# BerkIGuler/AdaFortiTran

Hardware: AMD Instinct MI355X
Metric: OFDM frames/sec (120x14 grid, batch 128) + channel-estimation MSE vs reference (higher is better)
Workload: dtype f32; 1 GPU; C3: AdaFortiTran default config (6 layers, d=128, 4 heads, adaptive tokens), 120x14 grid, pilots 12x2; 128 frames per GPU per step; step = model(pilots_cpu, meta_cpu) through the module surface + device MSE partial; value = SURVEY 8(d)'s metric: H2D of pilots + meta INSIDE the step, output left on the device (= value_h2d_inclusive); the bare engine call on inputs resident in HBM is value_resident;; frames_per_gpu=128, global_batch=128, parallelism=frames sharded over 1 rank(s), lanes=1

## Files before the change

adafortitran_amd/csrc/k_misc.hip:

```cpp
#include <algorithm>

#include "aft_internal.h"
#include "conv_device.h"
#include "pack_device.h"

namespace aft {

struct AdapterArgs {
    const float *cond[3];
    const float *w[3][3], *b[3][3];
    float *tokens6;
    int h0, h1, h2, tokens;
};

__device__ __forceinline__ void adapter_body(const AdapterArgs &a, int b, int e, float *sm) {
    float *a0 = sm, *a1 = sm + a.h0;
    const int tid = threadIdx.x;
    const float x = a.cond[e][b];
    constexpr int kH0Max = 8, kPer2 = 3;
    const bool fast = a.h0 <= kH0Max && a.h1 == 42 && a.h2 <= kPer2 * 256 && a.h1 <= 256;
    if (fast) {
        float w0 = 0.f, b0 = 0.f, w1[kH0Max], b1 = 0.f, b2[kPer2];
        f32x2 w2[kPer2][21];
        if (tid < a.h0) { w0 = a.w[e][0][tid]; b0 = a.b[e][0][tid]; }
#pragma unroll
        for (int k = 0; k < kH0Max; ++k) w1[k] = (tid < a.h1 && k < a.h0) ? a.w[e][1][tid * a.h0 + k] : 0.f;
        if (tid < a.h1) b1 = a.b[e][1][tid];
#pragma unroll
        for (int u = 0; u < kPer2; ++u) {
            const int i = tid + 256 * u;
            const bool ok = i < a.h2;
            const float *wr = a.w[e][2] + (size_t)(ok ? i : 0) * 42;
#pragma unroll
            for (int k = 0; k < 21; ++k) w2[u][k] = *reinterpret_cast<const f32x2 *>(wr + 2 * k);
            b2[u] = ok ? a.b[e][2][i] : 0.f;
        }
        if (tid < a.h0) a0[tid] = fmaxf(fmaf(w0, x, b0), 0.f);
        __syncthreads();
        if (tid < a.h1) {
            float acc = b1;
#pragma unroll
            for (int k = 0; k < kH0Max; ++k)
                if (k < a.h0) acc = fmaf(w1[k], a0[k], acc);
            a1[tid] = fmaxf(acc, 0.f);
        }
        __syncthreads();
#pragma unroll
        for (int u = 0; u < kPer2; ++u) {
            const int i = tid + 256 * u;
            if (i >= a.h2) break;
            float acc = b2[u];
#pragma unroll
            for (int k = 0; k < 21; ++k) {
                acc = fmaf(w2[u][k][0], a1[2 * k], acc);
                acc = fmaf(w2[u][k][1], a1[2 * k + 1], acc);
            }
            a.tokens6[((size_t)b * a.tokens + (i >> 1)) * 6 + 2 * e + (i & 1)] = acc;
        }
        return;
    }
    for (int i = tid; i < a.h0; i += 256) a0[i] = fmaxf(fmaf(a.w[e][0][i], x, a.b[e][0][i]), 0.f);
    __syncthreads();
    for (int i = tid; i < a.h1; i += 256) {
        float acc = a.b[e][1][i];
        for (int k = 0; k < a.h0; ++k) acc = fmaf(a.w[e][1][i * a.h0 + k], a0[k], acc);
        a1[i] = fmaxf(acc, 0.f);
    }
    __syncthreads();
    for (int i = tid; i < a.h2; i += 256) {
        float acc = a.b[e][2][i];
        const float *wr = a.w[e][2] + (size_t)i * a.h1;
        for (int k = 0; k < a.h1; ++k) acc = fmaf(wr[k], a1[k], acc);
        a.tokens6[((size_t)b * a.tokens + (i >> 1)) * 6 + 2 * e + (i & 1)] = acc;
    }
}

__global__ __launch_bounds__(256) void adapter_kernel(const AdapterArgs a) {
    extern __shared__ float sm[];
    adapter_body(a, blockIdx.x, blockIdx.y, sm);
}

static AdapterArgs adapter_args(const aft_config &c, const WeightsDev &w, const float *snr, const float *ds,
                                const float *dop, float *tokens6) {
    AdapterArgs a{};
    a.cond[0] = snr; a.cond[1] = ds; a.cond[2] = dop;
    for (int e = 0; e < 3; ++e)
        for (int j = 0; j < 3; ++j) { a.w[e][j] = w.ada_w[e][j]; a.b[e][j] = w.ada_b[e][j]; }
    a.tokens6 = tokens6;
    a.h0 = c.hidden[0]; a.h1 = c.hidden[1]; a.h2 = c.hidden[2];
    a.tokens = (c.num_scs / c.patch_scs) * (c.num_symbols / c.patch_symbols);
    return a;
}

hipError_t launch_adapter(const aft_config &c, const WeightsDev &w, const float *snr, const float *ds,
                          const float *dop, float *tokens6, int batch, hipStream_t st) {
    const AdapterArgs a = adapter_args(c, w, snr, ds, dop, tokens6);
    hipLaunchKernelGGL(adapter_kernel, dim3(batch, 3), dim3(256), sizeof(float) * (a.h0 + a.h1), st, a);
    return hipGetLastError();
}


constexpr int kFoldTok = 2, kFoldChunk = 16;
struct FoldArgs {
    const float *wkv, *bv;
    const float *w1, *b1, *pos;
    float *tk, *tvt, *wf;
    int d, K, tokens, tokpad;
};
inline size_t fold_tables_lds(int d) { return sizeof(float) * ((size_t)256 * (kFoldChunk + 1) + (size_t)kFoldTok * d); }

__device__ __forceinline__ void fold_tables_body(const FoldArgs &f, int blk, float *sm) {
    float *sw = sm, *sc = sm + 256 * (kFoldChunk + 1);
    const int tid = threadIdx.x, chunks = (2 * f.d + 255) / 256;
    const int t0 = (blk / chunks) * kFoldTok, row0 = (blk % chunks) * 256, row = row0 + tid;
    for (int i = tid; i < kFoldTok * f.d; i += 256) {
        const int tt = i / f.d, k = i - tt * f.d, t = t0 + tt;
        sc[i] = t < f.tokens ? f.b1[k] + f.pos[(size_t)t * f.d + k] : 0.f;
    }
    float acc[kFoldTok];
#pragma unroll
    for (int tt = 0; tt < kFoldTok; ++tt) acc[tt] = row >= f.d && row < 2 * f.d ? f.bv[row - f.d] : 0.f;
    constexpr int kPieces = kFoldChunk / 4;
    f32x4 piece[kPieces];
    auto request = [&](int kc) {
#pragma unroll
        for (int m = 0; m < kPieces; ++m) {
            const int i = tid + 256 * m, rr = i / kPieces, c4 = (i % kPieces) * 4;
            piece[m] = f32x4{0.f, 0.f, 0.f, 0.f};
            if (row0 + rr < 2 * f.d) piece[m] = *reinterpret_cast<const f32x4 *>(f.wkv + (size_t)(row0 + rr) * f.d + kc + c4);
        }
    };
    request(0);
    for (int kc = 0; kc < f.d; kc += kFoldChunk) {
        __syncthreads();
#pragma unroll
        for (int m = 0; m < kPieces; ++m) {
            const int i = tid + 256 * m, rr = i / kPieces, c4 = (i % kPieces) * 4;
#pragma unroll
            for (int j = 0; j < 4; ++j) sw[rr * (kFoldChunk + 1) + c4 + j] = piece[m][j];
        }
        if (kc + kFoldChunk < f.d) request(kc + kFoldChunk);
        __syncthreads();
#pragma unroll
        for (int kk = 0; kk < kFoldChunk; ++kk) {
            const float wv = sw[tid * (kFoldChunk + 1) + kk];
#pragma unroll
            for (int tt = 0; tt < kFoldTok; ++tt) acc[tt] = fmaf(wv, sc[tt * f.d + kc + kk], acc[tt]);
        }
    }
#pragma unroll
    for (int tt = 0; tt < kFoldTok; ++tt) {
        const int t = t0 + tt;
        if (row < f.d) {
            if (t < f.tokens) f.tk[(size_t)t * f.d + row] = acc[tt];
        } else if (row < 2 * f.d && t < f.tokpad) {
            f.tvt[(size_t)(row - f.d) * f.tokpad + t] = t < f.tokens ? acc[tt] : 0.f;
        }
    }
}

__device__ __forceinline__ void fold_matrices_body(const FoldArgs &f, int blk) {
    const int o = blk * 256 + threadIdx.x, per_part = (f.d / 32) * kFoldSteps * 64;
    if (o >= 2 * per_part) return;
    const int part = o / per_part, rem = o - part * per_part;
    const int wblock = rem / (kFoldSteps * 64), st = rem / 64 % kFoldSteps, lane = rem & 63;
    const int row = part * f.d + 32 * wblock + (lane & 31), k = 2 * st + (lane >> 5);
    float acc = 0.f;
    if (k < f.K) {
        const float *wr = f.wkv + (size_t)row * f.d;
        for (int j = 0; j < f.d; j += 4) {
            const f32x4 wv = *reinterpret_cast<const f32x4 *>(wr + j);
#pragma unroll
            for (int jj = 0; jj < 4; ++jj) acc = fmaf(wv[jj], f.w1[(size_t)(j + jj) * f.K + k], acc);
        }
    }
    f.wf[o] = acc;
}

struct PrologueArgs {
    AdapterArgs ad;
    float *packed;
    const float *pilots;
    float *up_planes;
    int adapter_blocks, pack_blocks, d, num_layers, split;
    int up_bx, npix, pf, nplanes;
    float *conv_frag;
    int frag_blocks;
    FoldArgs fold;
    int fold_table_blocks, fold_matrix_blocks;
};

__global__ __launch_bounds__(256) void prologue_kernel(const WeightsDev w, const PrologueArgs a) {
    extern __shared__ __attribute__((aligned(16))) float sm[];
    int blk = blockIdx.x;
    if (blk < a.adapter_blocks) {
        adapter_body(a.ad, blk / 3, blk % 3, sm);
        return;
    }
    blk -= a.adapter_blocks;
    if (blk < a.fold_table_blocks) {
        fold_tables_body(a.fold, blk, sm);
        return;
    }
    blk -= a.fold_table_blocks;
    if (blk < a.fold_matrix_blocks) {
        fold_matrices_body(a.fold, blk);
        return;
    }
    blk -= a.fold_matrix_blocks;
    if (blk < a.pack_blocks) {
        const size_t v = (size_t)blk * 256 + threadIdx.x, dd4 = (size_t)a.d * a.d / 4;
        if (a.fold_table_blocks > 0 && v >= dd4 && v < 3 * dd4) return;
        pack_weights_vec(w, a.packed, a.d, 0, a.num_layers, a.split, v);
        return;
    }
    blk -= a.pack_blocks;
    if (blk < a.frag_blocks) {
        const int v = blk * 256 + threadIdx.x;
        constexpr int kPerStack = kFragFloats / 4;
        if (v < 2 * kPerStack) {
            const int stack = v / kPerStack, rem = v - stack * kPerStack;
            const float *const *cw = stack ? w.ref_w : w.enh_w;
            const float *const *cb = stack ? w.ref_b : w.enh_b;
            f32x4 o;
            if (rem < kFragQuads * 64) {
                const int quad = rem >> 6, lane = rem & 63;
#pragma unroll
                for (int jj = 0; jj < 4; ++jj) o[jj] = conv_frag16_entry(cw[1], cb[1], cw[2], cb[2], 4 * quad + jj, lane);
            } else {
                const int i0 = 4 * (rem - kFragQuads * 64), h = i0 / 80;
#pragma unroll
                for (int jj = 0; jj < 4; ++jj) o[jj] = conv_helper_entry(cw[0], cb[0], cw[3], cb[3], h, i0 - 80 * h + jj);
            }
            *reinterpret_cast<f32x4 *>(a.conv_frag + (size_t)v * 4) = o;
        }
        return;
    }
    blk -= a.frag_blocks;
    upsample_planes_body(sm, w.up_w, w.up_b, a.pilots, a.up_planes, a.npix, a.pf, a.nplanes, blk % a.up_bx, blk / a.up_bx);
}

bool prologue_upsample_ok(const aft_config &c, const WeightsDev &w) {
    return upsample_planes_ok(w.up_w, c.pilot_scs * c.pilot_symbols);
}

hipError_t launch_prologue(const aft_config &c, const WeightsDev &w, const float *snr, const float *ds, const float *dop,
                           float *tokens6, int batch, float *packed, const float *pilots, float *up_planes, hipStream_t st,
                           float *conv_frag, const L0Fold *fold) {
    PrologueArgs a{};
    if (conv_frag != nullptr) {
        a.conv_frag = conv_frag;
        a.frag_blocks = (2 * (kFragFloats / 4) + 255) / 256;
    }
    size_t lds = 0;
    if (c.adaptive) {
        a.ad = adapter_args(c, w, snr, ds, dop, tokens6);
        a.adapter_blocks = 3 * batch;
        lds = sizeof(float) * (a.ad.h0 + a.ad.h1);
    }
    if (packed != nullptr) {
        a.packed = packed; a.d = c.model_dim; a.num_layers = std::min(c.num_layers, kLayerWindow);
        a.split = c.precision == AFT_PRECISION_BF16X3 ? 1 : 0;
        a.pack_blocks = (int)((packed_layer_floats(c.model_dim) * a.num_layers / 4 + 255) / 256);
    }
    int up_blocks = 0;
    if (up_planes != nullptr && prologue_upsample_ok(c, w)) {
        a.pilots = pilots; a.up_planes = up_planes;
        a.npix = c.num_scs * c.num_symbols; a.pf = c.pilot_scs * c.pilot_symbols; a.nplanes = 2 * batch;
        a.up_bx = (a.npix + kUpPix - 1) / kUpPix;
        up_blocks = a.up_bx * ((a.nplanes + kUpPlanes - 1) / kUpPlanes);
        lds = std::max(lds, upsample_planes_lds(a.pf));
    }
    if (fold != nullptr && fold->tk != nullptr) {
        FoldArgs &f = a.fold;
        f.d = c.model_dim; f.K = c.patch_scs * c.patch_symbols + (c.adaptive ? 6 : 0);
        f.tokens = tokens_of(c); f.tokpad = round_up(f.tokens, kTile);
        f.wkv = w.layers[0].in_proj_w + (size_t)f.d * f.d; f.bv = w.layers[0].in_proj_b + 2 * f.d;
        f.w1 = w.lin1_w; f.b1 = w.lin1_b; f.pos = w.pos;
        f.tk = fold->tk; f.tvt = fold->tvt; f.wf = fold->wf;
        a.d = c.model_dim;
        a.fold_table_blocks = (f.tokpad + kFoldTok - 1) / kFoldTok * ((2 * f.d + 255) / 256);
        a.fold_matrix_blocks = (2 * (f.d / 32) * kFoldSteps * 64 + 255) / 256;
        lds = std::max(lds, fold_tables_lds(f.d));
    }
    const int blocks = a.adapter_blocks + a.fold_table_blocks + a.fold_matrix_blocks + a.pack_blocks + a.frag_blocks + up_blocks;
    if (blocks == 0) return hipSuccess;
    hipLaunchKernelGGL(prologue_kernel, dim3(blocks), dim3(256), lds, st, w, a);
    return hipGetLastError();
}

struct EmbedArgs {
    const float *conv_enhanced, *tokens6, *w1, *b1, *pos;
    float *x;
    int S, T, p0, p1, tokens, d, din, planes;
};

template <int D, bool ADAPTIVE, int PMAX>
__global__ __launch_bounds__(256) void embed_kernel(const EmbedArgs a) {
    constexpr int PER = D / 32, NF = ADAPTIVE ? PMAX + 6 : PMAX;
    const int tid = threadIdx.x, hw = tid >> 5, lane32 = tid & 31;
    const int tw = a.T / a.p1, p = a.p0 * a.p1;
    extern __shared__ float sm[];
    for (int i = tid; i < a.din * D; i += 256) sm[(i % a.din) * D + i / a.din] = a.w1[i];
    __syncthreads();
    float w[NF][PER], b1[PER];
#pragma unroll
    for (int f = 0; f < NF; ++f) {
        const int frow = f < PMAX ? f : p + (f - PMAX);
#pragma unroll
        for (int i = 0; i < PER; ++i) w[f][i] = (f < PMAX && f >= p) ? 0.f : sm[frow * D + lane32 * PER + i];
    }
#pragma unroll
    for (int i = 0; i < PER; ++i) b1[i] = a.b1[lane32 * PER + i];
    const unsigned rows = (unsigned)a.planes * a.tokens, rstep = gridDim.x * 8u, tokens = a.tokens;
    const unsigned dn = rstep / tokens, dt = rstep % tokens;
    int poff[PMAX];
#pragma unroll
    for (int f = 0; f < PMAX; ++f) poff[f] = (f / a.p1) * a.T + f % a.p1;
    struct Tok { unsigned row, n, t; };
    auto advance = [&](Tok k) {
        k.row += rstep; k.n += dn; k.t += dt;
        if (k.t >= tokens) { k.t -= tokens; ++k.n; }
        return k;
    };
    auto fetch = [&](const Tok &k, float (&vin)[NF], float (&ps)[PER]) {
        const unsigned tq = k.t / (unsigned)tw, tr = k.t - tq * tw;
        const float *ce = a.conv_enhanced + ((size_t)k.n * a.S + tq * a.p0) * a.T + tr * a.p1;
#pragma unroll
        for (int f = 0; f < PMAX; ++f) vin[f] = f < p ? ce[poff[f]] : 0.f;
        if constexpr (ADAPTIVE) {
            const float *tk = a.tokens6 + ((size_t)(k.n >> 1) * tokens + k.t) * 6;
#pragma unroll
            for (int f = 0; f < 6; ++f) vin[PMAX + f] = tk[f];
        }
#pragma unroll
        for (int i = 0; i < PER; ++i) ps[i] = a.pos[k.t * D + lane32 * PER + i];
    };
    auto emit = [&](const Tok &k, const float (&vin)[NF], const float (&ps)[PER]) {
        float acc[PER];
#pragma unroll
        for (int i = 0; i < PER; ++i) acc[i] = b1[i] + ps[i];
#pragma unroll
        for (int f = 0; f < NF; ++f)
#pragma unroll
            for (int i = 0; i < PER; ++i) acc[i] = fmaf(w[f][i], vin[f], acc[i]);
#pragma unroll
        for (int i = 0; i < PER; ++i) a.x[(size_t)k.row * D + lane32 * PER + i] = acc[i];
    };
    float va[NF], pa[PER], vb[NF], pb[PER];
    Tok k0;
    k0.row = blockIdx.x * 8u + hw;
    k0.n = k0.row / tokens;
    k0.t = k0.row - k0.n * tokens;
    if (k0.row < rows) fetch(k0, va, pa);
    while (k0.row < rows) {
        const Tok k1 = advance(k0), k2 = advance(k1);
        if (k1.row < rows) fetch(k1, vb, pb);
        emit(k0, va, pa);
        if (k1.row < rows) {
            if (k2.row < rows) fetch(k2, va, pa);
            emit(k1, vb, pb);
        }
        k0 = k2;
    }
}

hipError_t launch_embed(const aft_config &c, const WeightsDev &w, const float *conv_enhanced, const float *tokens6,
                        float *x, int batch, hipStream_t st) {
    EmbedArgs a{};
    a.conv_enhanced = conv_enhanced; a.tokens6 = tokens6;
    a.w1 = w.lin1_w; a.b1 = w.lin1_b; a.pos = w.pos; a.x = x;
    a.S = c.num_scs; a.T = c.num_symbols; a.p0 = c.patch_scs; a.p1 = c.patch_symbols;
    a.tokens = (a.S / a.p0) * (a.T / a.p1);
    a.d = c.model_dim;
    a.din = a.p0 * a.p1 + (c.adaptive ? 6 : 0);
    a.planes = 2 * batch;
    const long rows = (long)a.planes * a.tokens;
    const int blocks = (int)std::min<long>((rows + 7) / 8, 1024);
    const size_t lds = sizeof(float) * a.din * a.d;
    const bool small = a.p0 * a.p1 <= 6;
    if (a.p0 * a.p1 > kMaxPatchFeatures) return hipErrorInvalidValue;
#define AFT_EMBED(D_, A_)                                                                              \
    do {                                                                                               \
        if (small) hipLaunchKernelGGL((embed_kernel<D_, A_, 6>), dim3(blocks), dim3(256), lds, st, a); \
        else hipLaunchKernelGGL((embed_kernel<D_, A_, kMaxPatchFeatures>), dim3(blocks), dim3(256), lds, st, a); \
    } while (0)
    if (c.model_dim == 32 && c.adaptive) AFT_EMBED(32, true);
    else if (c.model_dim == 32) AFT_EMBED(32, false);
    else if (c.model_dim == 96 && c.adaptive) AFT_EMBED(96, true);
    else if (c.model_dim == 96) AFT_EMBED(96, false);
    else if (c.model_dim == 160 && c.adaptive) AFT_EMBED(160, true);
    else if (c.model_dim == 160) AFT_EMBED(160, false);
    else if (c.model_dim == 224 && c.adaptive) AFT_EMBED(224, true);
    else if (c.model_dim == 224) AFT_EMBED(224, false);
    else if (c.model_dim == 64 && c.adaptive) AFT_EMBED(64, true);
    else if (c.model_dim == 64) AFT_EMBED(64, false);
    else if (c.model_dim == 128 && c.adaptive) AFT_EMBED(128, true);
    else if (c.model_dim == 128) AFT_EMBED(128, false);
    else if (c.model_dim == 192 && c.adaptive) AFT_EMBED(192, true);
    else if (c.model_dim == 192) AFT_EMBED(192, false);
    else if (c.model_dim == 256 && c.adaptive) AFT_EMBED(256, true);
    else if (c.model_dim == 256) AFT_EMBED(256, false);
    else return hipErrorInvalidValue;
#undef AFT_EMBED
    return hipGetLastError();
}

__global__ __launch_bounds__(256) void linear_kernel(const float *__restrict__ w, const float *__restrict__ bias,
                                                     const float *__restrict__ pilots, float *__restrict__ out,
                                                     int in_f, int out_f) {
    extern __shared__ float sm[];
    const int b = blockIdx.y;
    for (int i = threadIdx.x; i < 2 * in_f; i += 256) sm[i] = pilots[(size_t)b * 2 * in_f + i];
    __syncthreads();
    const int o = blockIdx.x * 256 + threadIdx.x;
    if (o >= out_f) return;
    const float bv = bias != nullptr ? bias[o] : 0.f;
    float re = bv, im = bv;
    const float *wr = w + (size_t)o * in_f;
    for (int k = 0; k < in_f; ++k) {
        re = fmaf(wr[k], sm[2 * k], re);
        im = fmaf(wr[k], sm[2 * k + 1], im);
    }
    *reinterpret_cast<float2 *>(out + ((size_t)b * out_f + o) * 2) = make_float2(re, im);
}

hipError_t launch_linear(const float *weight, const float *bias, const float *pilots, float *out, int batch,
                         int in_features, int out_features, hipStream_t st) {
    hipLaunchKernelGGL(linear_kernel, dim3((out_features + 255) / 256, batch), dim3(256),
                       sizeof(float) * 2 * in_features, st, weight, bias, pilots, out, in_features, out_features);
    return hipGetLastError();
}

__global__ __launch_bounds__(256) void mse_kernel(const float *__restrict__ est, const float *__restrict__ ref,
                                                  double *sum_sq, long long n_floats) {
    double acc = 0.0;
    const long long n4 = n_floats / 4;
    const long long stride = (long long)gridDim.x * 256;
    for (long long i = (long long)blockIdx.x * 256 + threadIdx.x; i < n4; i += stride) {
        const f32x4 e = reinterpret_cast<const f32x4 *>(est)[i];
        const f32x4 r = reinterpret_cast<const f32x4 *>(ref)[i];
#pragma unroll
        for (int j = 0; j < 4; ++j) {
            const float dlt = e[j] - r[j];
            acc += (double)dlt * (double)dlt;
        }
    }
    if (blockIdx.x == 0)
        for (long long i = n4 * 4 + threadIdx.x; i < n_floats; i += 256) {
            const float dlt = est[i] - ref[i];
            acc += (double)dlt * (double)dlt;
        }
#pragma unroll
    for (int o = 32; o >= 1; o >>= 1) acc += __shfl_xor(acc, o);
    __shared__ double part[4];
    if ((threadIdx.x & 63) == 0) part[threadIdx.x >> 6] = acc;
    __syncthreads();
    if (threadIdx.x == 0) atomicAdd(sum_sq, part[0] + part[1] + part[2] + part[3]);
}

hipError_t launch_mse(const float *est, const float *ref, double *sum_sq, long long n_complex, hipStream_t st) {
    const long long n_floats = 2 * n_complex;
    long long blocks = (n_floats / 4 + 255) / 256;
    if (blocks < 1) blocks = 1;
    if (blocks > 128) blocks = 128;
    hipLaunchKernelGGL(mse_kernel, dim3((int)blocks), dim3(256), 0, st, est, ref, sum_sq, n_floats);
    return hipGetLastError();
}

__global__ __launch_bounds__(256) void pilot_gather_kernel(const float2 *__restrict__ grid, float2 *__restrict__ pilots,
                                                           int *__restrict__ counts, int batch, int n, int expected) {
    const int lane = threadIdx.x & 63;
    const int frame = blockIdx.x * 4 + (threadIdx.x >> 6);
    if (frame >= batch) return;
    const float2 *src = grid + (size_t)frame * n;
    int base = 0;
    for (int i0 = 0; i0 < n; i0 += 8 * 64) {
        float2 v[8];
#pragma unroll
        for (int u = 0; u < 8; ++u) {
            const int i = i0 + 64 * u + lane;
            v[u] = i < n ? src[i] : make_float2(0.f, 0.f);
        }
#pragma unroll
        for (int u = 0; u < 8; ++u) {
            const bool nz = v[u].x != 0.f || v[u].y != 0.f;
            const unsigned long long m = __ballot(nz);
            const int pos = base + __popcll(m & ((1ull << lane) - 1ull));
            if (nz && pos < expected) pilots[(size_t)frame * expected + pos] = v[u];
            base += __popcll(m);
        }
    }
    for (int pos = base + lane; pos < expected; pos += 64)
        pilots[(size_t)frame * expected + pos] = make_float2(0.f, 0.f);
    if (lane == 0) counts[frame] = base;
}

hipError_t launch_pilot_gather(const float *hzero_ls, float *pilots, int *counts, int batch, int grid_elems,
                               int expected, hipStream_t st) {
    hipLaunchKernelGGL(pilot_gather_kernel, dim3((batch + 3) / 4), dim3(256), 0, st,
                       reinterpret_cast<const float2 *>(hzero_ls), reinterpret_cast<float2 *>(pilots), counts, batch,
                       grid_elems, expected);
    return hipGetLastError();
}

constexpr int kGatherLoads = 4, kGatherPiece = 64 * kGatherLoads;

struct FrameGatherArgs {
    const float *src[2];
    float *dst[2];
    const long long *index;
    int *flags;
    long long frames;
    unsigned waves, per_frame;
    int elems[2];
    int nvec[2], pieces[2];
    int wide[2];
};

template <typename V>
__device__ __forceinline__ void gather_piece(const float *src, float *dst, int nvec, int piece, int lane, bool ok) {
    V *d = reinterpret_cast<V *>(dst);
    const int i0 = piece * kGatherPiece + lane;
    if (ok) {
        const V *s = reinterpret_cast<const V *>(src);
        V v[kGatherLoads];
#pragma unroll
        for (int u = 0; u < kGatherLoads; ++u) v[u] = s[min(i0 + 64 * u, nvec - 1)];
#pragma unroll
        for (int u = 0; u < kGatherLoads; ++u) {
            const int i = i0 + 64 * u;
            if (i < nvec) d[i] = v[u];
        }
    } else {
#pragma unroll
        for (int u = 0; u < kGatherLoads; ++u) {
            const int i = i0 + 64 * u;
            if (i < nvec) d[i] = V{};
        }
    }
}

__global__ __launch_bounds__(256) void frame_gather_kernel(const FrameGatherArgs a) {
    const int lane = threadIdx.x & 63;
    const unsigned wave = __builtin_amdgcn_readfirstlane((int)(threadIdx.x >> 6)) + blockIdx.x * (blockDim.x >> 6);
    if (wave >= a.waves) return;
    const unsigned b = wave / a.per_frame;
    int piece = (int)(wave - b * a.per_frame);
    const int arr = piece < a.pieces[0] ? 0 : 1;
    if (arr) piece -= a.pieces[0];
    const long long idx = a.index[b];
    const bool ok = (unsigned long long)idx < (unsigned long long)a.frames;
    if (arr == 0 && piece == 0 && lane == 0) a.flags[b] = ok ? 0 : 1;
    const size_t fl = 2 * (size_t)a.elems[arr];
    const float *src = a.src[arr] + (ok ? (size_t)idx * fl : 0);
    float *dst = a.dst[arr] + (size_t)b * fl;
    if (a.wide[arr]) gather_piece<f32x4>(src, dst, a.nvec[arr], piece, lane, ok);
    else gather_piece<f32x2>(src, dst, a.nvec[arr], piece, lane, ok);
}

hipError_t launch_frame_gather(const float *ideal_all, const float *pilots_all, const long long *index, float *ideal_out,
                               float *pilots_out, int *flags, int batch, long long frames, int grid_elems, int pilot_elems,
                               hipStream_t st) {
    FrameGatherArgs a{};
    a.src[0] = ideal_all; a.src[1] = pilots_all; a.dst[0] = ideal_out; a.dst[1] = pilots_out;
    a.index = index; a.flags = flags; a.frames = frames;
    a.elems[0] = grid_elems; a.elems[1] = pilot_elems;
    for (int k = 0; k < 2; ++k) {
        const bool wide = a.elems[k] % 2 == 0 && (reinterpret_cast<uintptr_t>(a.src[k]) | reinterpret_cast<uintptr_t>(a.dst[k])) % 16 == 0;
        a.wide[k] = wide ? 1 : 0;
        a.nvec[k] = wide ? a.elems[k] / 2 : a.elems[k];
        a.pieces[k] = (a.nvec[k] + kGatherPiece - 1) / kGatherPiece;
    }
    a.per_frame = (unsigned)(a.pieces[0] + a.pieces[1]);
    const long long waves = (long long)batch * a.per_frame;
    if (waves > 0x7fffffffLL) return hipErrorInvalidValue;
    a.waves = (unsigned)waves;
    const int wpb = waves < 4LL * current_device_cus() ? 1 : 4;
    const long long blocks = (waves + wpb - 1) / wpb;
    hipLaunchKernelGGL(frame_gather_kernel, dim3((unsigned)blocks), dim3(64 * wpb), 0, st, a);
    return hipGetLastError();
}

constexpr int kEmbAnyRows = 8, kEmbAnyDin = kMaxPatchGeneral + 6;
__global__ __launch_bounds__(256) void embed_any_kernel(const EmbedArgs a) {
    __shared__ float in[kEmbAnyRows][kEmbAnyDin];
    const int tid = threadIdx.x, tw = a.T / a.p1, p = a.p0 * a.p1;
    const long rows = (long)a.planes * a.tokens, row0 = (long)blockIdx.x * kEmbAnyRows;
    for (int i = tid; i < kEmbAnyRows * kEmbAnyDin; i += 256) {
        const int r = i / kEmbAnyDin, f = i - r * kEmbAnyDin;
        const long row = row0 + r;
        float v = 0.f;
#ifdef AFT_TEST_LDS_BUG
        if (f >= a.din) continue;
#endif
        if (row < rows && f < a.din) {
            const int n = (int)(row / a.tokens), t = (int)(row - (long)n * a.tokens);
            if (f < p) {
                const int tq = t / tw, tr = t - tq * tw;
                v = a.conv_enhanced[((size_t)n * a.S + tq * a.p0 + f / a.p1) * a.T + tr * a.p1 + f % a.p1];
            } else {
                v = a.tokens6[((size_t)(n >> 1) * a.tokens + t) * 6 + (f - p)];
            }
        }
        in[r][f] = v;
    }
    __syncthreads();
    for (int c = tid; c < a.d; c += 256) {
        float w[kEmbAnyDin];
#pragma unroll
        for (int f = 0; f < kEmbAnyDin; ++f) w[f] = f < a.din ? a.w1[(size_t)c * a.din + f] : 0.f;
        const float b = a.b1[c];
        for (int r = 0; r < kEmbAnyRows; ++r) {
            const long row = row0 + r;
            if (row >= rows) break;
            const int t = (int)(row % a.tokens);
            float acc = b + a.pos[(size_t)t * a.d + c];
#pragma unroll
            for (int f = 0; f < kEmbAnyDin; ++f) acc = fmaf(w[f], in[r][f], acc);
            a.x[(size_t)row * a.d + c] = acc;
        }
    }
}

hipError_t launch_embed_any(const aft_config &c, const WeightsDev &w, const float *conv_enhanced, const float *tokens6,
                            float *x, int batch, hipStream_t st) {
    EmbedArgs a{};
    a.conv_enhanced = conv_enhanced; a.tokens6 = tokens6;
    a.w1 = w.lin1_w; a.b1 = w.lin1_b; a.pos = w.pos; a.x = x;
    a.S = c.num_scs; a.T = c.num_symbols; a.p0 = c.patch_scs; a.p1 = c.patch_symbols;
    a.tokens = (a.S / a.p0) * (a.T / a.p1);
    a.d = c.model_dim;
    a.din = a.p0 * a.p1 + (c.adaptive ? 6 : 0);
    a.planes = 2 * batch;
    if (a.p0 * a.p1 > kMaxPatchGeneral || (c.adaptive && tokens6 == nullptr)) return hipErrorInvalidValue;
    if (!switch_on(SW_EMBED_ANY_OLD) && ends_train_ok(a.planes, a.S, a.T, a.p0, a.p1, a.d, c.adaptive != 0))
        return launch_embed_train_fwd(conv_enhanced, c.adaptive ? tokens6 : nullptr, w.lin1_w, w.lin1_b, w.pos, x, a.planes, a.S, a.T, a.p0,
                                      a.p1, a.d, st, true);
    const long rows = (long)a.planes * a.tokens;
    hipLaunchKernelGGL(embed_any_kernel, dim3((unsigned)((rows + kEmbAnyRows - 1) / kEmbAnyRows)), dim3(256), 0, st, a);
    return hipGetLastError();
}

__global__ __launch_bounds__(1024) void fill_lds_kernel(float value, float *sink) {
    extern __shared__ __attribute__((aligned(16))) float lds_all[];
    constexpr int kFloats = 160 * 1024 / 4;
    for (int i = threadIdx.x; i < kFloats; i += 1024) lds_all[i] = value;
    __syncthreads();
    const unsigned long long t0 = __builtin_amdgcn_s_memtime();
    while (__builtin_amdgcn_s_memtime() - t0 < 20000) __builtin_amdgcn_s_sleep(16);
    if (sink != nullptr && lds_all[(threadIdx.x * 977) % kFloats] == 12345.678f) *sink = 1.f;
}
__global__ __launch_bounds__(256) void peek_lds_kernel(float *__restrict__ out, int n) {
    extern __shared__ __attribute__((aligned(16))) float lds_peek[];
    for (int i = threadIdx.x; i < n; i += 256) out[(size_t)blockIdx.x * n + i] = lds_peek[i];
}
hipError_t launch_peek_lds(float *out, int workgroups, int n, hipStream_t st) {
    hipLaunchKernelGGL(peek_lds_kernel, dim3(workgroups), dim3(256), 40 * 1024, st, out, n);
    return hipGetLastError();
}
hipError_t launch_fill_lds(float value, hipStream_t st) {
    static PerDeviceOnce attr;
    hipError_t e = ensure_dynamic_lds(attr, reinterpret_cast<const void *>(fill_lds_kernel), 160 * 1024);
    if (e != hipSuccess) return e;
    hipLaunchKernelGGL(fill_lds_kernel, dim3(4 * current_device_cus()), dim3(1024), 160 * 1024, st, value, (float *)nullptr);
    return hipGetLastError();
}

__global__ __launch_bounds__(256) void ls_mse_db_kernel(const float2 *__restrict__ ls, const float2 *__restrict__ ideal,
                                                        float *__restrict__ db, int batch, int n) {
    const int lane = threadIdx.x & 63;
    const int frame = blockIdx.x * 4 + (threadIdx.x >> 6);
    if (frame >= batch) return;
    double acc = 0.0;
    for (int i = lane; i < n; i += 64) {
        const float2 a = ls[(size_t)frame * n + i], b = ideal[(size_t)frame * n + i];
        const double dr = (double)a.x - (double)b.x, di = (double)a.y - (double)b.y;
        acc += dr * dr + di * di;
    }
#pragma unroll
    for (int o = 32; o >= 1; o >>= 1) acc += __shfl_xor(acc, o);
    if (lane == 0) db[frame] = (float)(10.0 * log10(acc / (double)n));
}

hipError_t launch_ls_mse_db(const float *ls, const float *ideal, float *db, int batch, int grid_elems, hipStream_t st) {
    hipLaunchKernelGGL(ls_mse_db_kernel, dim3((batch + 3) / 4), dim3(256), 0, st, reinterpret_cast<const float2 *>(ls),
                       reinterpret_cast<const float2 *>(ideal), db, batch, grid_elems);
    return hipGetLastError();
}

}
```

adafortitran_amd/csrc/switches.h:

```cpp
#pragma once

#define AFT_SWITCHES(X) \
    X(LANES, "AFT_LANES", "1 = never split a forward into lanes; 2 .. 4 = always that many shares (header section \"Lanes\")") \
    X(L0_FOLD, "AFT_L0_FOLD", "0 = layer 0's keys and values by the model_dim-deep product over x0, not from the input features on the prologue's tables (DESIGN.md 4.1)") \
    X(LAYER_FUSED, "AFT_LAYER_FUSED", "0 = never the one-launch-per-layer sequence (k_layer.hip), 1 = wherever its shape is covered (default: where plane-aligned tiles add no round)") \
    X(PROLOGUE_NO_UP, "AFT_PROLOGUE_NO_UP", "measurement: the profiled prologue launch without the pilot upsampler product") \
    X(CONV_NSPLIT, "AFT_CONV_NSPLIT", "1 | 2 | 4 column ranges per plane in the streaming conv kernels (default: by the batch)") \
    X(CONV_BANDED, "AFT_CONV_BANDED", "the banded conv kernel instead of the column- / row-streaming ones") \
    X(CONV_COLUMN_TILES, "AFT_CONV_COLUMN_TILES", "the column-tiled conv path even where a band plan fits; n > 2 = at least n tiles per plane") \
    X(GEMM_BM, "AFT_GEMM_BM", "64 | 96: row tile of the training GEMM (default: by the shape)") \
    X(EMBED_ANY_OLD, "AFT_EMBED_ANY_OLD", "the general engine's own embedding kernel instead of the training path's") \
    X(EMBED_BWD_GENERIC, "AFT_EMBED_BWD_GENERIC", "the vector embedding backward instead of the MFMA one (model_dim 128)") \
    X(TRAIN_UNFUSED_FWD, "AFT_TRAIN_UNFUSED_FWD", "the launch sequence the fused forward chain of a training layer replaced") \
    X(TRAIN_UNFUSED_BWD, "AFT_TRAIN_UNFUSED_BWD", "the launch sequence the fused backward chain of a training layer replaced") \
    X(TRAIN_ATTN_BWD_SPLIT, "AFT_TRAIN_ATTN_BWD_SPLIT", "the two-pass attention backward instead of the one-pass kernel") \
    X(ATTN_BWD_GROUPS, "AFT_ATTN_BWD_GROUPS", "1 | 4 problems per workgroup of the one-pass attention backward (default: by shape)") \
    X(STAMPS, "AFT_STAMPS", "phase stamps printed on the host: the diag variant only (libaft_hip_diag.so, build.build_diag(): -DAFT_DIAG_STAMPS)") \
    X(ALLOW_COMPOSITE, "AFT_ALLOW_COMPOSITE", "1 = run a configuration the kernels do not cover on the PyTorch-ROCm composite") \
    X(TRAIN_NO_FUSED_ENDS, "AFT_TRAIN_NO_FUSED_ENDS", "training: PyTorch's unfold / cat / add around the dense ends, not fused") \
    X(TRAIN_NO_QKV_CHAIN, "AFT_TRAIN_NO_QKV_CHAIN", "training: every layer runs its own in-projection GEMM (no chained tapes)") \
    X(PRECISION, "AFT_PRECISION", "f32 | bf16x3: the estimators' default hip_precision") \
    X(ENCODER_PATH, "AFT_ENCODER_PATH", "auto | launches | plane: aft_config.encoder_path of every HipEngine (`plane`: retired, runs the launches)")

namespace aft {

enum Switch : int {
#define AFT_SWITCH_ID(id, name, purpose) SW_##id,
    AFT_SWITCHES(AFT_SWITCH_ID)
#undef AFT_SWITCH_ID
    kNumSwitches
};

bool switch_on(Switch s);
int switch_int(Switch s, int dflt);

}
```

Before: 85520 frames/s.

## Compute layer-0 fold tables and matrices with MFMA tiles in the prologue

```diff
diff --git a/adafortitran_amd/csrc/k_misc.hip b/adafortitran_amd/csrc/k_misc.hip
--- a/adafortitran_amd/csrc/k_misc.hip
+++ b/adafortitran_amd/csrc/k_misc.hip
@@ -177,6 +177,109 @@
     f.wf[o] = acc;
 }
 
+__device__ __forceinline__ f32x4 fold_steps_of(f32x4 x) {
+    using u32x2 = __attribute__((ext_vector_type(2))) unsigned;
+    unsigned r[4];
+#pragma unroll
+    for (int c = 0; c < 4; ++c) { const float v = x[c]; r[c] = __builtin_bit_cast(unsigned, v); }
+    u32x2 p = __builtin_amdgcn_permlane32_swap(r[0], r[2], false, false);
+    r[0] = p[0]; r[2] = p[1];
+    p = __builtin_amdgcn_permlane32_swap(r[1], r[3], false, false);
+    r[1] = p[0]; r[3] = p[1];
+    p = __builtin_amdgcn_permlane16_swap(r[0], r[1], false, false);
+    r[0] = p[0]; r[1] = p[1];
+    p = __builtin_amdgcn_permlane16_swap(r[2], r[3], false, false);
+    r[2] = p[0]; r[3] = p[1];
+    return f32x4{__builtin_bit_cast(float, r[0]), __builtin_bit_cast(float, r[1]), __builtin_bit_cast(float, r[2]), __builtin_bit_cast(float, r[3])};
+}
+
+template <int NS, bool TABLE>
+__device__ __forceinline__ f32x4 fold_chain(const float *ap, const float *bp, int bstep, const float *cp, f32x4 acc, int blocks) {
+    constexpr int NQ = NS / 4;
+    for (int kb = 0; kb < blocks; ++kb) {
+        f32x4 av[NQ], bw[NQ], cw[NQ];
+        float bs[NS];
+#pragma unroll
+        for (int j = 0; j < NQ; ++j) av[j] = *reinterpret_cast<const f32x4 *>(ap + 16 * j);
+        if constexpr (TABLE) {
+#pragma unroll
+            for (int j = 0; j < NQ; ++j) bw[j] = *reinterpret_cast<const f32x4 *>(bp + 16 * j);
+#pragma unroll
+            for (int j = 0; j < NQ; ++j) cw[j] = *reinterpret_cast<const f32x4 *>(cp + 16 * j);
+        } else {
+#pragma unroll
+            for (int s = 0; s < NS; ++s) bs[s] = bp[(size_t)s * bstep];
+        }
+        __builtin_amdgcn_sched_barrier(0);
+#pragma unroll
+        for (int j = 0; j < NQ; ++j) {
+            const f32x4 a4 = fold_steps_of(av[j]);
+            f32x4 b4;
+            if constexpr (TABLE) b4 = fold_steps_of(cw[j] + bw[j]);
+            else b4 = f32x4{bs[4 * j], bs[4 * j + 1], bs[4 * j + 2], bs[4 * j + 3]};
+#pragma unroll
+            for (int m = 0; m < 4; ++m) acc = __builtin_amdgcn_mfma_f32_16x16x4f32(a4[m], b4[m], acc, 0, 0, 0);
+        }
+        ap += 4 * NS; bp += TABLE ? (size_t)4 * NS : (size_t)NS * bstep; cp += 4 * NS;
+    }
+    return acc;
+}
+template <bool TABLE>
+__device__ __forceinline__ f32x4 fold_chain_d(int d, const float *ap, const float *bp, int bstep, const float *cp, f32x4 acc) {
+    switch (d >> 5) {
+        case 1: return fold_chain<8, TABLE>(ap, bp, bstep, cp, acc, 1);
+        case 2: return fold_chain<16, TABLE>(ap, bp, bstep, cp, acc, 1);
+        case 3: return fold_chain<24, TABLE>(ap, bp, bstep, cp, acc, 1);
+        case 4: return fold_chain<32, TABLE>(ap, bp, bstep, cp, acc, 1);
+        case 5: return fold_chain<20, TABLE>(ap, bp, bstep, cp, acc, 2);
+        case 6: return fold_chain<24, TABLE>(ap, bp, bstep, cp, acc, 2);
+        case 7: return fold_chain<28, TABLE>(ap, bp, bstep, cp, acc, 2);
+        default: return fold_chain<32, TABLE>(ap, bp, bstep, cp, acc, 2);
+    }
+}
+
+constexpr int kFoldWaves = 4, kFoldMatCols = (2 * kFoldSteps + 15) / 16;
+inline int fold_table_tiles(int d, int tokpad) { return (2 * d / 16) * (tokpad / 16); }
+inline int fold_matrix_tiles(int d) { return (2 * d / 16) * kFoldMatCols; }
+
+__device__ __forceinline__ void fold_table_tile(const FoldArgs &f, int tile) {
+    const int lane = threadIdx.x & 63, i16 = lane & 15, g4 = lane >> 4, nrt = 2 * f.d / 16;
+    if (tile >= nrt * (f.tokpad / 16)) return;
+    const int row0 = 16 * (tile % nrt), t0 = 16 * (tile / nrt), t = t0 + i16;
+    const bool vrows = row0 >= f.d;
+    if (t0 >= f.tokens && !vrows) return;
+    f32x4 acc = {0.f, 0.f, 0.f, 0.f};
+    if (t0 < f.tokens) {
+        if (vrows) {
+#pragma unroll
+            for (int v = 0; v < 4; ++v) acc[v] = f.bv[row0 - f.d + 4 * g4 + v];
+        }
+        acc = fold_chain_d<true>(f.d, f.wkv + (size_t)(row0 + i16) * f.d + 4 * g4, f.pos + (size_t)min(t, f.tokens - 1) * f.d + 4 * g4, 0, f.b1 + 4 * g4, acc);
+    }
+    if (!vrows) {
+        if (t < f.tokens) *reinterpret_cast<f32x4 *>(f.tk + (size_t)t * f.d + row0 + 4 * g4) = acc;
+    } else {
+#pragma unroll
+        for (int v = 0; v < 4; ++v) f.tvt[(size_t)(row0 - f.d + 4 * g4 + v) * f.tokpad + t] = t < f.tokens ? acc[v] : 0.f;
+    }
+}
+
+__device__ __forceinline__ void fold_matrix_tile(const FoldArgs &f, int tile) {
+    const int lane = threadIdx.x & 63, i16 = lane & 15, g4 = lane >> 4, nrt = 2 * f.d / 16;
+    if (tile >= nrt * kFoldMatCols) return;
+    const int row0 = 16 * (tile % nrt), k0 = 16 * (tile / nrt), k = k0 + i16;
+    f32x4 acc = {0.f, 0.f, 0.f, 0.f};
+    if (k0 < f.K)
+        acc = fold_chain_d<false>(f.d, f.wkv + (size_t)(row0 + i16) * f.d + 4 * g4, f.w1 + (size_t)g4 * f.K + min(k, f.K - 1), 4 * f.K, nullptr, acc);
+    if (k >= 2 * kFoldSteps) return;
+    const int part = row0 >= f.d ? 1 : 0, r0 = row0 - part * f.d + 4 * g4;
+#pragma unroll
+    for (int v = 0; v < 4; ++v) {
+        const int r = r0 + v;
+        f.wf[((size_t)(part * (f.d / 32) + r / 32) * kFoldSteps + (k >> 1)) * 64 + (r & 31) + 32 * (k & 1)] = k < f.K ? acc[v] : 0.f;
+    }
+}
+
 struct PrologueArgs {
     AdapterArgs ad;
     float *packed;
@@ -188,6 +291,7 @@
     int frag_blocks;
     FoldArgs fold;
     int fold_table_blocks, fold_matrix_blocks;
+    int fold_legacy;
 };
 
 __global__ __launch_bounds__(256) void prologue_kernel(const WeightsDev w, const PrologueArgs a) {
@@ -199,12 +303,14 @@
     }
     blk -= a.adapter_blocks;
     if (blk < a.fold_table_blocks) {
-        fold_tables_body(a.fold, blk, sm);
+        if (a.fold_legacy) fold_tables_body(a.fold, blk, sm);
+        else fold_table_tile(a.fold, blk * kFoldWaves + __builtin_amdgcn_readfirstlane((int)(threadIdx.x >> 6)));
         return;
     }
     blk -= a.fold_table_blocks;
     if (blk < a.fold_matrix_blocks) {
-        fold_matrices_body(a.fold, blk);
+        if (a.fold_legacy) fold_matrices_body(a.fold, blk);
+        else fold_matrix_tile(a.fold, blk * kFoldWaves + __builtin_amdgcn_readfirstlane((int)(threadIdx.x >> 6)));
         return;
     }
     blk -= a.fold_matrix_blocks;
@@ -248,6 +354,7 @@
                            float *tokens6, int batch, float *packed, const float *pilots, float *up_planes, hipStream_t st,
                            float *conv_frag, const L0Fold *fold) {
     PrologueArgs a{};
+    const bool legacy = switch_on(SW_PROLOGUE_LEGACY);
     if (conv_frag != nullptr) {
         a.conv_frag = conv_frag;
         a.frag_blocks = (2 * (kFragFloats / 4) + 255) / 256;
@@ -279,9 +386,15 @@
         f.w1 = w.lin1_w; f.b1 = w.lin1_b; f.pos = w.pos;
         f.tk = fold->tk; f.tvt = fold->tvt; f.wf = fold->wf;
         a.d = c.model_dim;
-        a.fold_table_blocks = (f.tokpad + kFoldTok - 1) / kFoldTok * ((2 * f.d + 255) / 256);
-        a.fold_matrix_blocks = (2 * (f.d / 32) * kFoldSteps * 64 + 255) / 256;
-        lds = std::max(lds, fold_tables_lds(f.d));
+        a.fold_legacy = legacy || ((reinterpret_cast<uintptr_t>(f.b1) | reinterpret_cast<uintptr_t>(f.pos)) & 15) != 0 ? 1 : 0;
+        if (a.fold_legacy) {
+            a.fold_table_blocks = (f.tokpad + kFoldTok - 1) / kFoldTok * ((2 * f.d + 255) / 256);
+            a.fold_matrix_blocks = (2 * (f.d / 32) * kFoldSteps * 64 + 255) / 256;
+            lds = std::max(lds, fold_tables_lds(f.d));
+        } else {
+            a.fold_table_blocks = (fold_table_tiles(f.d, f.tokpad) + kFoldWaves - 1) / kFoldWaves;
+            a.fold_matrix_blocks = (fold_matrix_tiles(f.d) + kFoldWaves - 1) / kFoldWaves;
+        }
     }
     const int blocks = a.adapter_blocks + a.fold_table_blocks + a.fold_matrix_blocks + a.pack_blocks + a.frag_blocks + up_blocks;
     if (blocks == 0) return hipSuccess;
diff --git a/adafortitran_amd/csrc/switches.h b/adafortitran_amd/csrc/switches.h
--- a/adafortitran_amd/csrc/switches.h
+++ b/adafortitran_amd/csrc/switches.h
@@ -4,6 +4,7 @@
     X(LANES, "AFT_LANES", "1 = never split a forward into lanes; 2 .. 4 = always that many shares (header section \"Lanes\")") \
     X(L0_FOLD, "AFT_L0_FOLD", "0 = layer 0's keys and values by the model_dim-deep product over x0, not from the input features on the prologue's tables (DESIGN.md 4.1)") \
     X(LAYER_FUSED, "AFT_LAYER_FUSED", "0 = never the one-launch-per-layer sequence (k_layer.hip), 1 = wherever its shape is covered (default: where plane-aligned tiles add no round)") \
+    X(PROLOGUE_LEGACY, "AFT_PROLOGUE_LEGACY", "1 = the prologue launch's table and matrix bodies that the MFMA tiles replaced (A/B, tests; same bits)") \
     X(PROLOGUE_NO_UP, "AFT_PROLOGUE_NO_UP", "measurement: the profiled prologue launch without the pilot upsampler product") \
     X(CONV_NSPLIT, "AFT_CONV_NSPLIT", "1 | 2 | 4 column ranges per plane in the streaming conv kernels (default: by the batch)") \
     X(CONV_BANDED, "AFT_CONV_BANDED", "the banded conv kernel instead of the column- / row-streaming ones") \
```

New measurement: 85680 frames/s, median of 4. No clear change (+0.2%).
